# feiyeha/BS-YOLO

Measured on AMD Instinct MI355X. Metric: images/sec YOLO11s 640x640 bs=64 (forward + NMS), higher is better.
Workload: dtype f16

## Files before the change

bs_yolo_amd/csrc/conv_kernels.h:

```cpp
#pragma once
#include "common.h"

struct ConvK {
    const half_t* src0;
    const half_t* src1;
    int ld0, ld1, C0, C1, up0, up1;
    int H, W, OH, OW, stride, pad;
    int M;
    int Cin8;
    int ntaps;
    int nk;
    int Kpad;
    const half_t* wgt;
    const float* bias;
    void* dst;
    int ldd, Cout, out_f32;
    const half_t* res;
    int ldr;
    int act;
    int dst_scale, dst_dy, dst_dx;
    int ntn;
    int ntm;
    int tiles_x, tiles_y, B;
    int epi, y_f32, A, a0, nrows, raw_f32, rawC;
    float lvl_stride;
    int xyxy;
    void* y;
    void* raw;
    const half_t* tail_wgt;
    const float* tail_bias;
    unsigned span0, span1, wspan;
    int nsl_c, nsl_t, cb_per, taps_per, ldw;
    float* split_ws;
    long long slab;
    int korder;
};

__device__ __forceinline__ void dma16(const void* g, half_t* lds_wave_base) {
#if defined(__HIP_DEVICE_COMPILE__)
    __builtin_amdgcn_global_load_lds(g, lds_wave_base, 16, 0, 0);
#else
    (void)g;
    (void)lds_wave_base;
#endif
}

#if defined(__HIP_DEVICE_COMPILE__)
__device__ __forceinline__ void dma16_buf(bsy_rsrc_t r, unsigned voff, unsigned soff, half_t* lds_wave_base) {
    __builtin_amdgcn_raw_ptr_buffer_load_lds(r, lds_wave_base, 16, (int)voff, (int)soff, 0, 0);
}
#else
__device__ __forceinline__ void dma16_buf(bsy_rsrc_t, unsigned, unsigned, half_t*) {}
#endif

template <int MT, int NT>
__device__ __forceinline__ void conv_epilogue(const ConvK& p, f32x16 (&acc)[NT][MT], int m0, int n0, int wm, int wn,
                                              int lrow, int lh) {
    const int ohw = p.OH * p.OW;
    const bool wide = !p.out_f32 && !(p.Cout & 15) && !(p.ldd & 7) && !((uintptr_t)p.dst & 15);
#pragma unroll
    for (int b = 0; b < MT; ++b) {
        const int m = m0 + (wm * MT + b) * 32 + lrow;
        const bool mvalid = m < p.M;
        size_t dpix = (size_t)(mvalid ? m : 0);
        if (p.dst_scale != 1) {
            const int mm = mvalid ? m : 0;
            const int n = mm / ohw;
            const int rem = mm - n * ohw;
            const int oh = rem / p.OW;
            const int ow = rem - oh * p.OW;
            dpix = ((size_t)n * (p.OH * p.dst_scale) + (oh * p.dst_scale + p.dst_dy)) * (size_t)(p.OW * p.dst_scale) +
                   (ow * p.dst_scale + p.dst_dx);
        }
#pragma unroll
        for (int a = 0; a < NT; ++a) {
            const int cbase = n0 + (wn * NT + a) * 32;
            if (cbase >= p.Cout) continue;
            if (wide) {
                unsigned pk[4][2];
#pragma unroll
                for (int g = 0; g < 4; ++g) {
                    const int c = cbase + 8 * g + 4 * lh;
                    float v[4] = {0.f, 0.f, 0.f, 0.f};
                    if (c < p.Cout) {
#pragma unroll
                        for (int e = 0; e < 4; ++e) {
                            float t = acc[a][b][4 * g + e];
                            v[e] = p.act ? silu_f(t) : t;
                        }
                        if (p.res && mvalid) {
                            const half4 rv = *reinterpret_cast<const half4*>(p.res + dpix * p.ldr + c);
#pragma unroll
                            for (int e = 0; e < 4; ++e) v[e] += (float)rv[e];
                        }
                    }
                    half2v h0 = {(half_t)v[0], (half_t)v[1]}, h1 = {(half_t)v[2], (half_t)v[3]};
                    pk[g][0] = __builtin_bit_cast(unsigned, h0);
                    pk[g][1] = __builtin_bit_cast(unsigned, h1);
                }
#pragma unroll
                for (int g = 0; g < 4; g += 2) {
                    const auto r0 = __builtin_amdgcn_permlane32_swap(pk[g][0], pk[g + 1][0], false, false);
                    const auto r1 = __builtin_amdgcn_permlane32_swap(pk[g][1], pk[g + 1][1], false, false);
                    const int c = cbase + 8 * (g + lh);
                    if (mvalid && c < p.Cout) {
                        uint4 o = {r0[0], r1[0], r0[1], r1[1]};
                        *reinterpret_cast<uint4*>(reinterpret_cast<half_t*>(p.dst) + dpix * p.ldd + c) = o;
                    }
                }
                continue;
            }
            if (!mvalid) continue;
#pragma unroll
            for (int g = 0; g < 4; ++g) {
                const int c = cbase + 8 * g + 4 * lh;
                if (c >= p.Cout) continue;
                float v[4];
#pragma unroll
                for (int e = 0; e < 4; ++e) {
                    float t = acc[a][b][4 * g + e];
                    if (p.act) t = silu_f(t);
                    v[e] = t;
                }
                const bool full = c + 3 < p.Cout;
                if (p.res) {
                    const half_t* rp = p.res + dpix * p.ldr + c;
                    if (full) {
                        const half4 rv = *reinterpret_cast<const half4*>(rp);
#pragma unroll
                        for (int e = 0; e < 4; ++e) v[e] += (float)rv[e];
                    } else {
#pragma unroll
                        for (int e = 0; e < 4; ++e)
                            if (c + e < p.Cout) v[e] += (float)rp[e];
                    }
                }
                if (p.out_f32) {
                    float* dp = reinterpret_cast<float*>(p.dst) + dpix * p.ldd + c;
                    if (full) {
                        f32x4 o = {v[0], v[1], v[2], v[3]};
                        *reinterpret_cast<f32x4*>(dp) = o;
                    } else {
#pragma unroll
                        for (int e = 0; e < 4; ++e)
                            if (c + e < p.Cout) dp[e] = v[e];
                    }
                } else {
                    half_t* dp = reinterpret_cast<half_t*>(p.dst) + dpix * p.ldd + c;
                    if (full) {
                        half4 o = {(half_t)v[0], (half_t)v[1], (half_t)v[2], (half_t)v[3]};
                        *reinterpret_cast<half4*>(dp) = o;
                    } else {
#pragma unroll
                        for (int e = 0; e < 4; ++e)
                            if (c + e < p.Cout) dp[e] = (half_t)v[e];
                    }
                }
            }
        }
    }
}

template <typename T>
__device__ __forceinline__ void head_store(void* base, size_t idx, float v) { reinterpret_cast<T*>(base)[idx] = (T)v; }

__device__ __forceinline__ void dfl_decode_store(const ConvK& p, const f32x16& lo, const f32x16& hi, bool mv,
                                                 size_t ybase, size_t rbase, int pix, int lh) {
    const int hw = p.OH * p.OW;
    float dist[4];
#pragma unroll
    for (int sd = 0; sd < 4; ++sd) {
        const int rb = 8 * (sd & 1);
        float v[8];
#pragma unroll
        for (int g = 0; g < 2; ++g)
#pragma unroll
            for (int e = 0; e < 4; ++e) v[4 * g + e] = ((sd >> 1) ? hi : lo)[rb + 4 * g + e];
        if (p.raw && mv) {
#pragma unroll
            for (int i = 0; i < 8; ++i) {
                const size_t ri = rbase + (size_t)(16 * sd + (i & 3) + 8 * (i >> 2) + 4 * lh) * hw;
                if (p.raw_f32) head_store<float>(p.raw, ri, v[i]); else head_store<half_t>(p.raw, ri, v[i]);
            }
        }
        float mx = v[0];
#pragma unroll
        for (int i = 1; i < 8; ++i) mx = fmaxf(mx, v[i]);
        mx = fmaxf(mx, __shfl_xor(mx, 32, 64));
        float den = 0.f, num = 0.f;
#pragma unroll
        for (int i = 0; i < 8; ++i) {
            const float ex = __expf(v[i] - mx);
            den += ex;
            num += ex * (float)((i & 3) + 8 * (i >> 2) + 4 * lh);
        }
        den += __shfl_xor(den, 32, 64);
        num += __shfl_xor(num, 32, 64);
        dist[sd] = num / den;
    }
    if (mv && lh == 0) {
        const int ay_i = pix / p.OW, ax_i = pix - ay_i * p.OW;
        const float ax = (float)ax_i + 0.5f, ay = (float)ay_i + 0.5f;
        const float x1 = ax - dist[0], y1 = ay - dist[1], x2 = ax + dist[2], y2 = ay + dist[3];
        const float o[4] = {(p.xyxy ? x1 : (x1 + x2) * 0.5f) * p.lvl_stride, (p.xyxy ? y1 : (y1 + y2) * 0.5f) * p.lvl_stride,
                            (p.xyxy ? x2 : x2 - x1) * p.lvl_stride, (p.xyxy ? y2 : y2 - y1) * p.lvl_stride};
#pragma unroll
        for (int r = 0; r < 4; ++r) {
            const size_t yi = ybase + (size_t)r * p.A;
            if (p.y_f32) head_store<float>(p.y, yi, o[r]); else head_store<half_t>(p.y, yi, o[r]);
        }
    }
}

template <int MT, int NT>
__device__ __forceinline__ void conv_epilogue_head(const ConvK& p, f32x16 (&acc)[NT][MT], int m0, int n0, int wm, int wn,
                                                   int lrow, int lh) {
    const int hw = p.OH * p.OW;
#pragma unroll
    for (int b = 0; b < MT; ++b) {
        const int m = m0 + (wm * MT + b) * 32 + lrow;
        const bool mv = m < p.M;
        const int mm = mv ? m : 0;
        const int n = mm / hw, pix = mm - n * hw;
        const size_t ybase = (size_t)n * p.nrows * p.A + p.a0 + pix;
        const size_t rbase = (size_t)n * p.rawC * hw + pix;
        if (p.epi == 2) {
#pragma unroll
            for (int a = 0; a < NT; ++a) {
                const int cl = n0 + (wn * NT + a) * 32;
                if (cl >= p.Cout) continue;
#pragma unroll
                for (int g = 0; g < 4; ++g) {
                    const int c0 = cl + 8 * g + 4 * lh;
#pragma unroll
                    for (int e = 0; e < 4; ++e) {
                        const int c = c0 + e;
                        if (!mv || c >= p.Cout) continue;
                        const float v = acc[a][b][4 * g + e];
                        const float sg = sigmoid_f(v);
                        const size_t yi = ybase + (size_t)(4 + c) * p.A;
                        if (p.y_f32) head_store<float>(p.y, yi, sg); else head_store<half_t>(p.y, yi, sg);
                        if (p.raw) {
                            const size_t ri = rbase + (size_t)(64 + c) * hw;
                            if (p.raw_f32) head_store<float>(p.raw, ri, v); else head_store<half_t>(p.raw, ri, v);
                        }
                    }
                }
            }
        } else if (NT == 2) {
            dfl_decode_store(p, acc[0][b], acc[NT - 1][b], mv, ybase, rbase, pix, lh);
        }
    }
}

template <int TM, int TN, int MT, int NT, int NTHR>
__device__ __forceinline__ void conv_epilogue_cls_lds(const ConvK& p, f32x16 (&acc)[NT][MT], half_t* stile, int m0, int n0,
                                                      int wm, int wn, int lrow, int lh, int tid) {
    constexpr int LDP = TM + 8;
#pragma unroll
    for (int b = 0; b < MT; ++b) {
        const int prow = (wm * MT + b) * 32 + lrow;
#pragma unroll
        for (int a = 0; a < NT; ++a) {
            const int cl = (wn * NT + a) * 32;
            if (n0 + cl >= p.Cout) continue;
#pragma unroll
            for (int g = 0; g < 4; ++g) {
                const int c = cl + 8 * g + 4 * lh;
#pragma unroll
                for (int e = 0; e < 4; ++e) {
                    const float v = acc[a][b][4 * g + e];
                    stile[(c + e) * LDP + prow] = (half_t)sigmoid_f(v);
                }
            }
        }
    }
    __syncthreads();
    const int hw = p.OH * p.OW;
    half_t* y = reinterpret_cast<half_t*>(p.y);
    constexpr int GPR = TM / 8;
    for (int id = tid; id < TN * GPR; id += NTHR) {
        const int cr = id / GPR, g8 = (id - cr * GPR) * 8;
        const int c = n0 + cr, m = m0 + g8;
        if (c >= p.Cout || m >= p.M) continue;
        const int n = m / hw, pix = m - n * hw;
        const size_t yi = ((size_t)n * p.nrows + 4 + c) * p.A + p.a0 + pix;
        if (pix + 8 <= hw && m + 8 <= p.M && !(yi & 7)) {
            *reinterpret_cast<half8*>(y + yi) = *reinterpret_cast<const half8*>(stile + cr * LDP + g8);
        } else {
            for (int e = 0; e < 8 && m + e < p.M; ++e) {
                const int me = m + e, ne = me / hw, pe = me - ne * hw;
                y[((size_t)ne * p.nrows + 4 + c) * p.A + p.a0 + pe] = stile[cr * LDP + g8 + e];
            }
        }
    }
}

template <int TM, int TN, int MT, int NT, int NTHR>
__device__ __forceinline__ void conv_epilogue_lds(const ConvK& p, f32x16 (&acc)[NT][MT], half_t* stile, int m0, int n0,
                                                  int wm, int wn, int lrow, int lh, int tid) {
    constexpr int LDT = TN + 8;
#pragma unroll
    for (int b = 0; b < MT; ++b) {
        const int prow = (wm * MT + b) * 32 + lrow;
#pragma unroll
        for (int a = 0; a < NT; ++a) {
            const int cl = (wn * NT + a) * 32;
#pragma unroll
            for (int g = 0; g < 4; ++g) {
                const int c = cl + 8 * g + 4 * lh;
                half4 o;
                f32x4 t = f32x4{acc[a][b][4 * g], acc[a][b][4 * g + 1], acc[a][b][4 * g + 2], acc[a][b][4 * g + 3]};
                if (p.act) t = silu4_f(t);
#pragma unroll
                for (int e = 0; e < 4; ++e) o[e] = (half_t)t[e];
                *reinterpret_cast<half4*>(stile + prow * LDT + c) = o;
            }
        }
    }
    __syncthreads();
    constexpr int CPRW = TN / 8;
    constexpr int ITER = TM * CPRW / NTHR;
    half_t* dst = reinterpret_cast<half_t*>(p.dst);
#pragma unroll
    for (int i = 0; i < ITER; ++i) {
        const int id = tid + NTHR * i;
        const int row = id / CPRW, cc = (id % CPRW) * 8;
        const int m = m0 + row, c = n0 + cc;
        if (m >= p.M || c >= p.Cout) continue;
        half8 v = *reinterpret_cast<const half8*>(stile + row * LDT + cc);
        if (p.res) {
            const half8 r = *reinterpret_cast<const half8*>(p.res + (size_t)m * p.ldr + c);
#pragma unroll
            for (int e = 0; e < 8; ++e) v[e] = (half_t)((float)v[e] + (float)r[e]);
        }
        *reinterpret_cast<half8*>(dst + (size_t)m * p.ldd + c) = v;
    }
}

int launch_gemm_cfg(int id, int ksize, const ConvK& k, hipStream_t s);
int launch_stream1x1_cfg(int id, const ConvK& k, hipStream_t s);
int launch_patch_cfg(int id, bool tail, const ConvK& k, hipStream_t s);

constexpr int PERSIST_MAX_COUT = 1024;
```

bs_yolo_amd/csrc/conv_select.hip:

```cpp
#include <stdlib.h>

#include "conv_kernels.h"

extern "C" int bsy_conv_packed_dims(int C2, int C1, int ksize, int* cout_pad, int* k_pad) {
    if (C2 <= 0 || C1 <= 0 || (ksize != 1 && ksize != 3)) BSY_FAIL(BSY_ERR_ARG, "conv_packed_dims: bad shape");
    if (cout_pad) *cout_pad = round_up(C2, 128);
    if (C1 == 3) C1 = 4;
    if (k_pad) *k_pad = round_up(ksize * ksize * C1, 32);
    return BSY_OK;
}

int conv_korder(const ConvArgs& a) {
    const int Cin = a.C0 + a.C1;
    if (a.ksize != 3 || (Cin & 31) || (a.C0 & 31)) return 0;
    return (a.stride == 2 && !(Cin & 63) && !(a.C0 & 63)) ? 2 : 1;
}

enum ConvFam { CONV_GEMM, CONV_PERSIST, CONV_WRES, CONV_PATCH, CONV_TAIL };
struct ConvCfg {
    int id; ConvFam fam;
    int tm, tn, stages, bk;
    bool aligned;
    int tw, nfr;
};
template <int WM, int WN, int MT, int NT, int S, bool AL, int BK> constexpr ConvCfg gemm_row(int id) {
    return {id, CONV_GEMM, WM * MT * 32, WN * NT * 32, S, BK, AL, 0, 0};
}
template <int WM, int WN, int MT, int NT, int S, int BK> constexpr ConvCfg persist_row(int id) {
    return {id, CONV_PERSIST, WM * MT * 32, WN * NT * 32, S, BK, true, 0, 0};
}
template <int NT, int S, int NFR> constexpr ConvCfg wres_row(int id) {
    return {id, CONV_WRES, 128, 64 * NT, S, 32, true, 0, NFR};
}
template <int NT, int S, int TW, bool TAIL = false> constexpr ConvCfg patch_row(int id) {
    return {id, TAIL ? CONV_TAIL : CONV_PATCH, TW == 16 ? 8 * 16 : 6 * 20, 64 * NT, S, 32, true, TW, 0};
}
static const ConvCfg kConvCfgs[] = {
    gemm_row<4, 1, 2, 1, 3, false, 32>(0x00),
    gemm_row<4, 1, 2, 1, 3, true, 32>(0x01),
    gemm_row<4, 1, 2, 1, 2, true, 32>(0x02),
    gemm_row<4, 1, 2, 1, 2, true, 64>(0x03),
    gemm_row<4, 1, 2, 2, 3, false, 32>(0x10),
    gemm_row<4, 1, 2, 2, 3, true, 32>(0x11),
    gemm_row<4, 1, 2, 2, 2, true, 32>(0x12),
    gemm_row<4, 1, 2, 2, 2, true, 64>(0x13),
    gemm_row<2, 2, 2, 2, 3, false, 32>(0x20),
    gemm_row<2, 2, 2, 2, 3, true, 32>(0x21),
    gemm_row<2, 2, 2, 2, 2, true, 32>(0x22),
    gemm_row<2, 2, 2, 2, 2, true, 64>(0x23),
    gemm_row<2, 2, 2, 1, 3, false, 32>(0x30),
    gemm_row<2, 2, 2, 1, 3, true, 32>(0x31),
    gemm_row<2, 2, 2, 1, 2, true, 32>(0x32),
    gemm_row<2, 2, 2, 1, 2, true, 64>(0x33),
    gemm_row<4, 2, 2, 2, 3, true, 32>(0x41),
    gemm_row<4, 2, 2, 2, 2, true, 32>(0x42),
    gemm_row<4, 2, 2, 2, 2, true, 64>(0x43),
    gemm_row<1, 4, 2, 1, 3, false, 32>(0x50),
    gemm_row<1, 4, 2, 1, 3, true, 32>(0x51),
    gemm_row<1, 4, 2, 1, 2, true, 32>(0x52),
    gemm_row<1, 4, 2, 1, 2, true, 64>(0x53),
    gemm_row<2, 2, 1, 1, 3, false, 32>(0x60),
    gemm_row<2, 2, 1, 1, 3, true, 32>(0x61),
    gemm_row<2, 2, 1, 1, 2, true, 32>(0x62),
    gemm_row<2, 2, 1, 1, 2, true, 64>(0x63),
    gemm_row<4, 2, 2, 4, 3, true, 32>(0x71),
    gemm_row<4, 2, 2, 4, 2, true, 32>(0x72),
    gemm_row<4, 2, 2, 4, 2, true, 64>(0x73),
    persist_row<2, 2, 2, 2, 3, 32>(0x81),
    persist_row<2, 2, 2, 2, 2, 32>(0x82),
    persist_row<2, 2, 2, 2, 2, 64>(0x83),
    persist_row<2, 2, 2, 1, 3, 32>(0x91),
    persist_row<2, 2, 2, 1, 2, 32>(0x92),
    persist_row<2, 2, 2, 1, 2, 64>(0x93),
    patch_row<2, 2, 16>(0xA1),
    patch_row<1, 3, 16>(0xB1),
    patch_row<1, 2, 16>(0xB2),
    patch_row<1, 4, 16>(0xB3),
    patch_row<2, 2, 20>(0xC1),
    patch_row<1, 3, 20>(0xD1),
    patch_row<1, 2, 20>(0xD2),
    patch_row<1, 4, 20>(0xD3),
    patch_row<1, 3, 16, true>(0xB1),
    patch_row<1, 2, 16, true>(0xB2),
    patch_row<1, 4, 16, true>(0xB3),
    patch_row<1, 3, 20, true>(0xD1),
    patch_row<1, 2, 20, true>(0xD2),
    patch_row<1, 4, 20, true>(0xD3),
    wres_row<2, 4, 24>(0xE1),
    wres_row<2, 3, 24>(0xE2),
    wres_row<1, 4, 32>(0xF1),
    wres_row<1, 3, 32>(0xF2),
};

static const ConvCfg* conv_cfg_row(int cfg, bool tail) {
    for (const ConvCfg& r : kConvCfgs) if (r.id == (cfg & ~4) && (r.fam == CONV_TAIL) == tail) return &r;
    return nullptr;
}

bool conv_cfg_valid(const ConvArgs& a, int cfg) {
    const ConvCfg* r = conv_cfg_row(cfg, a.tail_wgt != nullptr);
    if (!r) return false;
    const int Cin = a.C0 + a.C1, ko = conv_korder(a), nsl = a.nsl_c * a.nsl_t;
    const bool aligned = !(Cin & 31) && !(a.C0 & 31), aligned64 = !(Cin & 63) && !(a.C0 & 63);
    if ((r->aligned && !aligned) || (r->bk == 64 && !aligned64)) return false;
    if (r->fam == CONV_GEMM) {
        if (!(cfg & 4) != !ko) return false;
        if (ko && (!r->aligned || (ko == 1 && r->bk == 64))) return false;
        if (nsl > 1 && (!r->aligned || (Cin / (a.nsl_c > 0 ? a.nsl_c : 1)) % r->bk)) return false;
        if (a.epi == 3 && (r->tm != 256 || r->tn != 64)) return false;
        return r->tn != 256 || !(a.Cout & 255);
    }
    if ((cfg & 4) || nsl > 1 || (r->fam == CONV_TAIL ? (a.epi != 3 || a.Cout != 64 || a.res) : a.epi != 0)) return false;
    if (a.out_f32 || (a.Cout & 7) || (a.ldd & 7) || ((uintptr_t)a.dst & 15) || a.dst_scale > 1) return false;
    if (r->fam == CONV_PERSIST || r->fam == CONV_WRES) {
        if (a.ksize != 1 || a.stride != 1 || a.res) return false;
        if (r->fam == CONV_PERSIST) return a.Cout <= PERSIST_MAX_COUT;
        return (r->tn / 64) * (Cin / 16) <= r->nfr && Cin / 32 >= r->stages - 1 && (r->tn != 128 || a.Cout > 64);
    }
    return ko == 1 && a.ksize == 3 && a.stride == 1 && a.pad == 1 && !a.C1 && !a.up0 && (!a.res || (!(a.ldr & 7) && !((uintptr_t)a.res & 15))) &&
           (r->tn != 128 || a.Cout > 64);
}

static bool family_off(const char* env) { return getenv(env) != nullptr; }

int conv_candidates(const ConvArgs& a, int* out, int max_out) {
    const int Cin = a.C0 + a.C1;
    const bool aligned = !(Cin & 31) && !(a.C0 & 31), aligned64 = !(Cin & 63) && !(a.C0 & 63);
    const long long M = (long long)a.B * a.OH * a.OW;
    const int tile = a.epi == 3 ? 1 : (a.Cout > 64 ? 2 : (a.Cout > 32 ? 1 : 0));
    const int ko = conv_korder(a), km = ko ? 4 : 0;
    const bool t20 = ceil_div(a.W, 20) * ceil_div(a.H, 6) < ceil_div(a.W, 16) * ceil_div(a.H, 8);
    int n = 0;
    auto add = [&](int c) {
        for (int i = 0; i < n; ++i) if (out[i] == c) return;
        if (n < max_out && conv_cfg_valid(a, c)) out[n++] = c;
    };
    if (a.tail_wgt) {
        if (t20) { add(0xD2); add(0xD1); add(0xD3); }
        add(0xB2); add(0xB1); add(0xB3); add(0xD2); add(0xD1); add(0xD3);
        return n;
    }
    if (!aligned) {
        add(tile << 4);
        if (a.Cout > 32) { add(0x30); add(0x60); }
        if (a.Cout > 64) add(0x50);
        return n;
    }
    const bool patch_ok = !family_off("BSY_NO_PATCH");
    if (!a.epi && a.ksize == 3 && a.stride == 1 && a.H >= 16 && a.W >= 16 && patch_ok) add(t20 ? 0xD2 : 0xB2);
    const int vbest = (aligned64 && ko != 1) ? 3 : 1;
    if (!a.epi && !(a.Cout & 255) && aligned64 && ko != 1 && M >= 16384) add(0x73 | km);
    add(tile << 4 | vbest | km);
    for (const ConvCfg& r : kConvCfgs) {
        if ((r.fam != CONV_GEMM && r.fam != CONV_PERSIST) || !r.aligned) continue;
        if (r.tn >= 2 * round_up(a.Cout, 32)) continue;
        if (r.tn == 32 && a.Cout > 32) continue;
        if (r.tm == 256 && r.tn == 128 && (a.Cout < 128 || M < 32768)) continue;
        if (r.tn == 256 && M < 16384) continue;
        if (r.fam == CONV_PERSIST && (M < 65536 || family_off("BSY_NO_PERSIST"))) continue;
        add(r.id | (r.fam == CONV_GEMM ? km : 0));
    }
    if (a.ksize == 1 && M >= 65536 && !family_off("BSY_NO_WRES"))
        for (const ConvCfg& r : kConvCfgs) if (r.fam == CONV_WRES) add(r.id);
    if (a.H >= 16 && a.W >= 16 && patch_ok)
        for (const ConvCfg& r : kConvCfgs) if (r.fam == CONV_PATCH && (r.tw == 16 || t20)) add(r.id);
    return n;
}

int launch_conv(const ConvArgs& a, hipStream_t s) {
    const int Cin = a.C0 + a.C1;
    if (a.ksize != 1 && a.ksize != 3) BSY_FAIL(BSY_ERR_ARG, "conv: ksize %d unsupported", a.ksize);
    if (a.stride != 1 && a.stride != 2) BSY_FAIL(BSY_ERR_ARG, "conv: stride %d unsupported", a.stride);
    if ((a.C0 & 7) || (a.C1 & 7) || (a.ld0 & 7) || (a.C1 && (a.ld1 & 7)))
        BSY_FAIL(BSY_ERR_ARG, "conv: channel counts/strides must be multiples of 8 (C0=%d C1=%d ld0=%d ld1=%d)", a.C0,
                 a.C1, a.ld0, a.ld1);
    if ((a.ldd & 3) || (a.res && (a.ldr & 3))) BSY_FAIL(BSY_ERR_ARG, "conv: dst/res row stride must be a multiple of 4");
    if (((uintptr_t)a.src0 & 15) || ((uintptr_t)a.src1 & 15) || ((uintptr_t)a.wgt & 15) || ((uintptr_t)a.bias & 15) ||
        ((uintptr_t)a.dst & 7) || ((uintptr_t)a.res & 7))
        BSY_FAIL(BSY_ERR_ARG, "conv: misaligned pointer");
    if (a.C1 && !a.src1) BSY_FAIL(BSY_ERR_ARG, "conv: src1 missing");
    if ((a.up0 && ((a.H | a.W) & 1)) || (a.up1 && ((a.H | a.W) & 1))) BSY_FAIL(BSY_ERR_ARG, "conv: odd size with upsample");
    if (a.OH != (a.H + 2 * a.pad - a.ksize) / a.stride + 1 || a.OW != (a.W + 2 * a.pad - a.ksize) / a.stride + 1)
        BSY_FAIL(BSY_ERR_ARG, "conv: output extent mismatch");
    const long long M = (long long)a.B * a.OH * a.OW;
    if (M <= 0 || M > 0x7fffffffLL) BSY_FAIL(BSY_ERR_ARG, "conv: M out of range");
    if (a.epi) {
        if ((a.epi != 2 && a.epi != 3) || !a.y || a.A <= 0 || a.a0 < 0 || a.a0 + a.OH * a.OW > a.A || a.dst_scale > 1 || a.res)
            BSY_FAIL(BSY_ERR_ARG, "conv: bad fused-decoder arguments (epi %d)", a.epi);
        if (a.epi == 3 && (a.Cout != 64 || a.nrows < 4)) BSY_FAIL(BSY_ERR_ARG, "conv: DFL epilogue needs 64 box channels");
        if (a.tail_wgt && (a.epi != 3 || !a.tail_bias || a.ksize != 3 || ((uintptr_t)a.tail_wgt & 15) || ((uintptr_t)a.tail_bias & 15)))
            BSY_FAIL(BSY_ERR_ARG, "conv: bad box-branch tail arguments");
        if (a.epi == 2 && a.nrows < 4 + a.Cout) BSY_FAIL(BSY_ERR_ARG, "conv: y has %d rows, class epilogue needs %d", a.nrows, 4 + a.Cout);
        if (a.raw && a.rawC < (a.epi == 3 ? 64 : 64 + a.Cout)) BSY_FAIL(BSY_ERR_ARG, "conv: raw map has too few channels");
    }
    ConvK k;
    k.src0 = a.src0; k.src1 = a.src1; k.ld0 = a.ld0; k.ld1 = a.ld1; k.C0 = a.C0; k.C1 = a.C1;
    k.up0 = a.up0; k.up1 = a.up1; k.H = a.H; k.W = a.W; k.OH = a.OH; k.OW = a.OW; k.stride = a.stride; k.pad = a.pad;
    k.M = (int)M; k.Cin8 = Cin / 8; k.ntaps = a.ksize * a.ksize;
    k.Kpad = round_up(a.ksize * a.ksize * Cin, 32); k.nk = k.Kpad / 32;
    k.wgt = a.wgt; k.bias = a.bias; k.dst = a.dst; k.ldd = a.ldd; k.Cout = a.Cout; k.out_f32 = a.out_f32;
    k.res = a.res; k.ldr = a.ldr; k.act = a.act; k.B = a.B; k.tiles_x = k.tiles_y = 0;
    k.epi = a.epi; k.y = a.y; k.y_f32 = a.y_f32; k.A = a.A; k.a0 = a.a0; k.nrows = a.nrows; k.lvl_stride = a.lvl_stride;
    k.xyxy = a.epi == 3 && a.xyxy;
    k.raw = a.raw; k.raw_f32 = a.raw_f32; k.rawC = a.rawC;
    k.tail_wgt = a.tail_wgt; k.tail_bias = a.tail_bias;
    if (a.tail_wgt && !a.epi) BSY_FAIL(BSY_ERR_ARG, "conv: a box-branch tail needs the decoder arguments (epi 3)");
    k.dst_scale = a.dst_scale > 0 ? a.dst_scale : 1; k.dst_dy = a.dst_dy; k.dst_dx = a.dst_dx; k.ntn = 1;
    k.nsl_c = k.nsl_t = 1; k.cb_per = Cin; k.taps_per = a.ksize * a.ksize; k.split_ws = nullptr; k.slab = 0; k.ldw = 0;
    if (a.nsl_c * a.nsl_t > 1) {
        const int nt = a.ksize * a.ksize;
        if (a.nsl_c < 1 || a.nsl_t < 1 || !a.split_ws || a.epi || a.out_f32 || a.tail_wgt || (a.dst_scale > 1) || (Cin % a.nsl_c) || ((Cin / a.nsl_c) & 31) || (a.C0 & 31) ||
            (nt % a.nsl_t) || (a.Cout & 7) || (a.ldd & 7) || ((uintptr_t)a.dst & 15) || (a.res && ((a.ldr & 7) || ((uintptr_t)a.res & 15))) || ((uintptr_t)a.split_ws & 15))
            BSY_FAIL(BSY_ERR_ARG, "conv: bad split-K arguments (%d x %d slices)", a.nsl_c, a.nsl_t);
        if (conv_korder(a) == 2 && ((Cin / a.nsl_c) & 63)) BSY_FAIL(BSY_ERR_ARG, "conv: split-K slices of a 64-channel-chunk layer must be multiples of 64 channels");
        k.nsl_c = a.nsl_c; k.nsl_t = a.nsl_t; k.cb_per = Cin / a.nsl_c; k.taps_per = nt / a.nsl_t; k.split_ws = a.split_ws;
        k.ldw = round_up(a.Cout, 32);
        k.slab = (long long)M * k.ldw;
    }
    if (a.ksize == 3 && (a.up0 || a.up1)) BSY_FAIL(BSY_ERR_ARG, "conv: upsampled source only with ksize 1");
    if ((long long)a.B * a.H * a.W * (long long)(a.ld0 > a.ld1 ? a.ld0 : a.ld1) >= (1LL << 31))
        BSY_FAIL(BSY_ERR_ARG, "conv: source view exceeds 2^31 elements (split the batch)");
    {
        const long long px0 = (long long)a.B * (a.H >> a.up0) * (a.W >> a.up0), px1 = (long long)a.B * (a.H >> a.up1) * (a.W >> a.up1);
        k.span0 = (unsigned)(((px0 - 1) * a.ld0 + a.C0) * 2);
        k.span1 = a.C1 ? (unsigned)(((px1 - 1) * a.ld1 + a.C1) * 2) : 0u;
        k.wspan = (unsigned)((long long)round_up(a.Cout, 128) * k.Kpad * 2);
    }
    int cfg = a.cfg;
    if (cfg < 0 || !conv_cfg_valid(a, cfg)) {
        int list[BSY_CONV_MAX_CFG];
        if (conv_candidates(a, list, BSY_CONV_MAX_CFG) <= 0) BSY_FAIL(BSY_ERR_ARG, "conv: no kernel configuration for this shape");
        cfg = list[0];
    }
    k.korder = conv_korder(a);
    const ConvCfg* r = conv_cfg_row(cfg, a.tail_wgt != nullptr);
    switch (r->fam) {
        case CONV_GEMM: return launch_gemm_cfg(r->id, a.ksize, k, s);
        case CONV_PERSIST:
        case CONV_WRES: return launch_stream1x1_cfg(r->id, k, s);
        case CONV_PATCH:
        case CONV_TAIL: return launch_patch_cfg(r->id, r->fam == CONV_TAIL, k, s);
    }
    BSY_FAIL(BSY_ERR_ARG, "conv: configuration 0x%02x has no kernel family", cfg);
}
```

bs_yolo_amd/csrc/conv_stream1x1.hip:

```cpp
#include "conv_kernels.h"

template <int WAVES_M, int WAVES_N, int MT, int NT, int STAGES, int BK>
__global__ __launch_bounds__(512) void conv1x1_persist_kernel(const ConvK p) {
    constexpr int TM = WAVES_M * MT * 32, TN = WAVES_N * NT * 32;
    constexpr int TNS = TN < 64 ? 64 : TN;
    constexpr int CPR = BK / 8, RPI = 64 / CPR;
    constexpr int PIW = TM / (RPI * 4), WIW = TNS / (RPI * 4);
    constexpr int STAGE = (TM + TNS) * BK, NDMA = PIW + WIW;
    constexpr int SWS = BK == 32 ? 2 : 1;
    constexpr int LDT = TN + 8, OT = TM * LDT;
    static_assert(WAVES_M * WAVES_N == 4 && PIW >= 1 && WIW >= 1 && (BK == 32 || (!(PIW & 1) && !(WIW & 1))), "bad tile");
    __shared__ __attribute__((aligned(16))) half_t smem[STAGES * STAGE + OT + 2 * PERSIST_MAX_COUT];
    half_t* otile = smem + STAGES * STAGE;
    float* sbias = reinterpret_cast<float*>(otile + OT);

    const int tid = threadIdx.x, lane = tid & 63;
    const int wave = __builtin_amdgcn_readfirstlane(tid >> 6);
    const int nk = p.Kpad / BK;
    const int ntiles = p.ntm * p.ntn;
    const TileWalk tw = xcd_tile_walk(blockIdx.x, gridDim.x, ntiles);
    const int T0 = tw.tile, G = tw.step;
    const int my_tiles = T0 < tw.end ? (tw.end - T0 + G - 1) / G : 0;
    for (int i = tid; i < p.ntn * TN; i += 512) sbias[i] = p.bias[i];
    __syncthreads();

    if (wave >= 4) {
        const int st = tid - 256;
        constexpr int CPRW = TN / 8, ITER = TM * CPRW / 256;
        half_t* dst = reinterpret_cast<half_t*>(p.dst);
        for (int t = 0; t < my_tiles; ++t) {
            const int tile = T0 + t * G;
            const int m0 = (tile / p.ntn) * TM, n0 = (tile % p.ntn) * TN;
            for (int k = 0; k < nk; ++k) __builtin_amdgcn_s_barrier();
            __builtin_amdgcn_s_barrier();
            half8 v[ITER];
#pragma unroll
            for (int i = 0; i < ITER; ++i) {
                const int id = st + 256 * i;
                v[i] = *reinterpret_cast<const half8*>(otile + (id / CPRW) * LDT + (id % CPRW) * 8);
            }
#pragma unroll
            for (int i = 0; i < ITER; ++i) {
                const int id = st + 256 * i;
                const int m = m0 + id / CPRW, c = n0 + (id % CPRW) * 8;
                if (m < p.M && c < p.Cout) *reinterpret_cast<half8*>(dst + (size_t)m * p.ldd + c) = v[i];
            }
        }
        return;
    }

    const int wm = wave / WAVES_N, wn = wave % WAVES_N;
    const int rsub = lane / CPR, slot = lane % CPR;
    const int kc0 = BK == 32 ? (slot ^ ((rsub >> 2) & 3)) : (slot ^ (rsub >> 1));
    const int kc1 = BK == 32 ? kc0 : (slot ^ (4 | (rsub >> 1)));
    const bsy_rsrc_t rs0 = make_rsrc(p.src0, p.span0), rs1 = make_rsrc(p.src1 ? p.src1 : p.src0, p.src1 ? p.span1 : 0u),
                     rsw = make_rsrc(p.wgt, p.wspan);
    const int ohw = p.OH * p.OW;
    const int Cin = p.Cin8 * 8;

    unsigned off0[PIW], off1[PIW], woff[WIW];
    bool rv[PIW];
    int it = 0, ikt = 0, s_cb = 0;
    auto setup_tile = [&](int tcount) {
        const int tile = T0 + tcount * G;
        const int m0 = (tile / p.ntn) * TM, n0 = (tile % p.ntn) * TN;
#pragma unroll
        for (int i = 0; i < PIW; ++i) {
            const int m = m0 + (wave * PIW + i) * RPI + rsub;
            rv[i] = m < p.M;
            const int mm = rv[i] ? m : 0;
            if (!(p.up0 | p.up1) && p.stride == 1) {
                off0[i] = (unsigned)mm * (unsigned)p.ld0;
                off1[i] = (unsigned)mm * (unsigned)p.ld1;
            } else {
                const int n = mm / ohw, rem = mm - n * ohw, oh = rem / p.OW, ow = rem - oh * p.OW;
                const int iy = oh * p.stride, ix = ow * p.stride;
                const int H0 = p.H >> p.up0, W0 = p.W >> p.up0, H1 = p.H >> p.up1, W1 = p.W >> p.up1;
                off0[i] = (unsigned)((n * H0 + (iy >> p.up0)) * W0 + (ix >> p.up0)) * (unsigned)p.ld0;
                off1[i] = (unsigned)((n * H1 + (iy >> p.up1)) * W1 + (ix >> p.up1)) * (unsigned)p.ld1;
            }
        }
#pragma unroll
        for (int j = 0; j < WIW; ++j)
            woff[j] = (unsigned)(n0 + (wave * WIW + j) * RPI + rsub) * (unsigned)p.Kpad + ((j & 1) ? kc1 : kc0) * 8;
        s_cb = 0;
    };
    auto issue_step = [&](int stage) {
        if (ikt == 0) setup_tile(it);
        half_t* sP = smem + stage * STAGE;
        half_t* sW = sP + TM * BK;
        const bool s1 = s_cb >= p.C0;
        const unsigned sc = 2u * (unsigned)(s1 ? s_cb - p.C0 : s_cb);
#pragma unroll
        for (int i = 0; i < PIW; ++i) {
            const unsigned kcb = 16u * (unsigned)((i & 1) ? kc1 : kc0);
            const unsigned o = rv[i] ? 2u * (s1 ? off1[i] : off0[i]) + sc + kcb : BSY_OOB;
            if (s1) dma16_buf(rs1, o, 0u, sP + (wave * PIW + i) * RPI * BK);
            else dma16_buf(rs0, o, 0u, sP + (wave * PIW + i) * RPI * BK);
        }
#pragma unroll
        for (int j = 0; j < WIW; ++j)
            dma16_buf(rsw, 2u * woff[j], (unsigned)ikt * (2u * BK), sW + (wave * WIW + j) * RPI * BK);
        s_cb += BK;
        if (++ikt == nk) { ikt = 0; ++it; }
    };

    const int lrow = lane & 31, lh = lane >> 5;
    f32x16 acc[NT][MT];
#pragma unroll
    for (int a = 0; a < NT; ++a)
#pragma unroll
        for (int b = 0; b < MT; ++b) acc_bias(acc[a][b], sbias + (T0 % p.ntn) * TN + (wn * NT + a) * 32, lh);
    const int total = my_tiles * nk;
    int ip = 0;
    for (; ip < STAGES - 1 && ip < total; ++ip) issue_step(ip % STAGES);
    int ckt = 0, ct = 0;
    for (int cp = 0; cp < total; ++cp) {
        const int later = min(STAGES - 2, total - 1 - cp);
        if (later >= STAGES - 2 && STAGES > 2) {
            asm volatile("s_waitcnt vmcnt(%0)" ::"n"((STAGES - 2) * NDMA) : "memory");
        } else {
            asm volatile("s_waitcnt vmcnt(0)" ::: "memory");
        }
        __builtin_amdgcn_s_barrier();
        if (ip < total) { issue_step(ip % STAGES); ++ip; }
        const half_t* sP = smem + (cp % STAGES) * STAGE;
        const half_t* sW = sP + TM * BK;
        constexpr int KSUB = BK / 16;
        half8 bfr[KSUB][MT], afr[KSUB][NT];
#pragma unroll
        for (int ks = 0; ks < KSUB; ++ks) {
            const int chunk = 2 * ks + lh;
#pragma unroll
            for (int b = 0; b < MT; ++b) {
                const int row = (wm * MT + b) * 32 + lrow;
                bfr[ks][b] = *reinterpret_cast<const half8*>(sP + row * BK + ((chunk ^ ((row >> SWS) & (CPR - 1))) << 3));
            }
#pragma unroll
            for (int a = 0; a < NT; ++a) {
                const int row = (wn * NT + a) * 32 + lrow;
                afr[ks][a] = *reinterpret_cast<const half8*>(sW + row * BK + ((chunk ^ ((row >> SWS) & (CPR - 1))) << 3));
            }
        }
        __builtin_amdgcn_sched_barrier(0);
#pragma unroll
        for (int ks = 0; ks < KSUB; ++ks)
#pragma unroll
            for (int a = 0; a < NT; ++a)
#pragma unroll
                for (int b = 0; b < MT; ++b)
                    acc[a][b] = __builtin_amdgcn_mfma_f32_32x32x16_f16(afr[ks][a], bfr[ks][b], acc[a][b], 0, 0, 0);
        if (++ckt == nk) {
            ckt = 0;
            const int n1 = ((T0 + (ct + 1) * G) % p.ntn) * TN;
#pragma unroll
            for (int b = 0; b < MT; ++b) {
                const int prow = (wm * MT + b) * 32 + lrow;
#pragma unroll
                for (int a = 0; a < NT; ++a) {
                    const int cl = (wn * NT + a) * 32;
#pragma unroll
                    for (int g = 0; g < 4; ++g) {
                        const int c = cl + 8 * g + 4 * lh;
                        const f32x4 bn = *reinterpret_cast<const f32x4*>(sbias + n1 + c);
                        half4 o;
                        f32x4 tv = f32x4{acc[a][b][4 * g], acc[a][b][4 * g + 1], acc[a][b][4 * g + 2], acc[a][b][4 * g + 3]};
                        if (p.act) tv = silu4_f(tv);
#pragma unroll
                        for (int e = 0; e < 4; ++e) {
                            o[e] = (half_t)tv[e];
                            acc[a][b][4 * g + e] = bn[e];
                        }
                        *reinterpret_cast<half4*>(otile + prow * LDT + c) = o;
                    }
                }
            }
            asm volatile("s_waitcnt lgkmcnt(0)" ::: "memory");
            __builtin_amdgcn_s_barrier();
            ++ct;
        }
    }
}

template <int WM, int WN, int MT, int NT, int STAGES, int BK>
static int launch_persist(const ConvK& k, hipStream_t s) {
    constexpr int TM = WM * MT * 32, TN = WN * NT * 32;
    ConvK p = k;
    p.ntn = ceil_div(k.Cout, TN);
    p.ntm = ceil_div(k.M, TM);
    const long long ntiles = (long long)p.ntm * p.ntn;
    if (ntiles <= 0 || ntiles > 0x7fffffffLL) BSY_FAIL(BSY_ERR_ARG, "conv: tile count %lld out of range", ntiles);
    constexpr int lds_bytes = ((TM + (TN < 64 ? 64 : TN)) * BK * STAGES + TM * (TN + 8) + 2 * PERSIST_MAX_COUT) * 2;
    const int per_cu = 160 * 1024 / lds_bytes > 2 ? 2 : (160 * 1024 / lds_bytes);
    const long long grid = ntiles < 256LL * per_cu ? ntiles : 256LL * per_cu;
    hipLaunchKernelGGL((conv1x1_persist_kernel<WM, WN, MT, NT, STAGES, BK>), dim3((unsigned)grid), dim3(512), 0, s, p);
    HIP_TRY(hipGetLastError());
    return BSY_OK;
}

template <int NT, int STAGES, int NFR>
__global__ __launch_bounds__(256, 2) void conv1x1_wres_kernel(const ConvK p) {
    constexpr int BK = 32, MT = 2, TM = 128, TN = 64 * NT;
    constexpr int CPR = 4, RPI = 16;
    constexpr int PIW = TM / (RPI * 4);
    constexpr int STAGE = TM * BK;
    constexpr int LDT = TN + 8, OT = TM * LDT;
    constexpr int CPRW = TN / 8, NST = TM * CPRW / 256;
    __shared__ __attribute__((aligned(16))) half_t smem[STAGES * STAGE + OT + 2 * TN];
    half_t* otile = smem + STAGES * STAGE;
    float* sbias = reinterpret_cast<float*>(otile + OT);

    const int tid = threadIdx.x, lane = tid & 63;
    const int wave = __builtin_amdgcn_readfirstlane(tid >> 6);
    const int wm = wave >> 1, wn = wave & 1;
    const int lrow = lane & 31, lh = lane >> 5;
    const int nk = p.Kpad / BK;
    constexpr int X = 8;
    const int x = blockIdx.x % X, q = blockIdx.x / X;
    const int ct = q % p.ntn, slot = q / p.ntn;
    const int walkers = (gridDim.x / X) / p.ntn;
    const int per = p.ntm / X, rem = p.ntm % X;
    const int pt0 = x * per + (x < rem ? x : rem), ptn = per + (x < rem ? 1 : 0);
    const int my_tiles = slot < ptn ? (ptn - slot + walkers - 1) / walkers : 0;
    const int n0 = ct * TN;

    half8 afr[NFR];
    const int nfr = nk * 2 * NT;
#pragma unroll
    for (int i = 0; i < NFR; ++i) {
        afr[i] = half8{0, 0, 0, 0, 0, 0, 0, 0};
        if (i < nfr) {
            const int ks = i / NT, a = i - ks * NT;
            afr[i] = *reinterpret_cast<const half8*>(p.wgt + (size_t)(n0 + (wn * NT + a) * 32 + lrow) * p.Kpad + 16 * ks + 8 * lh);
        }
    }
    if (tid < TN) sbias[tid] = p.bias[n0 + tid];
    asm volatile("s_waitcnt vmcnt(0)" ::: "memory");
    __syncthreads();

    const int rsub = lane / CPR, slot4 = lane % CPR;
    const int kc = slot4 ^ ((rsub >> 2) & 3);
    const bsy_rsrc_t rs0 = make_rsrc(p.src0, p.span0), rs1 = make_rsrc(p.src1 ? p.src1 : p.src0, p.src1 ? p.span1 : 0u);
    const int ohw = p.OH * p.OW;
    unsigned off0[PIW], off1[PIW];
    bool rv[PIW];
    int it = 0, ikt = 0, s_cb = 0;
    auto setup_tile = [&](int tcount) {
        const int m0 = (pt0 + slot + tcount * walkers) * TM;
#pragma unroll
        for (int i = 0; i < PIW; ++i) {
            const int m = m0 + (wave * PIW + i) * RPI + rsub;
            rv[i] = m < p.M;
            const int mm = rv[i] ? m : 0;
            if (!(p.up0 | p.up1)) {
                off0[i] = (unsigned)mm * (unsigned)p.ld0;
                off1[i] = (unsigned)mm * (unsigned)p.ld1;
            } else {
                const int n = mm / ohw, r2 = mm - n * ohw, oh = r2 / p.OW, ow = r2 - oh * p.OW;
                const int H0 = p.H >> p.up0, W0 = p.W >> p.up0, H1 = p.H >> p.up1, W1 = p.W >> p.up1;
                off0[i] = (unsigned)((n * H0 + (oh >> p.up0)) * W0 + (ow >> p.up0)) * (unsigned)p.ld0;
                off1[i] = (unsigned)((n * H1 + (oh >> p.up1)) * W1 + (ow >> p.up1)) * (unsigned)p.ld1;
            }
        }
        s_cb = 0;
    };
    auto issue_step = [&](int stage) {
        if (ikt == 0) setup_tile(it);
        half_t* sP = smem + stage * STAGE;
        const bool s1 = s_cb >= p.C0;
        const unsigned sc = 2u * (unsigned)(s1 ? s_cb - p.C0 : s_cb) + 16u * (unsigned)kc;
#pragma unroll
        for (int i = 0; i < PIW; ++i) {
            const unsigned o = rv[i] ? 2u * (s1 ? off1[i] : off0[i]) + sc : BSY_OOB;
            if (s1) dma16_buf(rs1, o, 0u, sP + (wave * PIW + i) * RPI * BK);
            else dma16_buf(rs0, o, 0u, sP + (wave * PIW + i) * RPI * BK);
        }
        s_cb += BK;
        if (++ikt == nk) { ikt = 0; ++it; }
    };

    f32x16 acc[NT][MT];
#pragma unroll
    for (int a = 0; a < NT; ++a)
#pragma unroll
        for (int b = 0; b < MT; ++b) acc_bias(acc[a][b], sbias + (wn * NT + a) * 32, lh);
    const int total = my_tiles * nk;
    int ip = 0;
    for (; ip < STAGES - 1 && ip < total; ++ip) issue_step(ip % STAGES);
    int ckt = 0, ct_done = 0;
    half_t* dst = reinterpret_cast<half_t*>(p.dst);
    for (int cp = 0; cp < total; ++cp) {
        const int later = min(STAGES - 2, total - 1 - cp);
        const bool st_young = ct_done > 0 && ckt < STAGES - 1;
        if (later >= STAGES - 2) {
            if (st_young) asm volatile("s_waitcnt vmcnt(%0)" ::"n"((STAGES - 2) * PIW + NST) : "memory");
            else asm volatile("s_waitcnt vmcnt(%0)" ::"n"((STAGES - 2) * PIW) : "memory");
        } else {
            asm volatile("s_waitcnt vmcnt(0)" ::: "memory");
        }
        __builtin_amdgcn_s_barrier();
        if (ip < total) { issue_step(ip % STAGES); ++ip; }
        const half_t* sP = smem + (cp % STAGES) * STAGE;
#pragma unroll
        for (int ks = 0; ks < 2; ++ks) {
            const int chunk = 2 * ks + lh;
            half8 bfr[MT];
#pragma unroll
            for (int b = 0; b < MT; ++b) {
                const int row = (wm * MT + b) * 32 + lrow;
                bfr[b] = *reinterpret_cast<const half8*>(sP + row * BK + ((chunk ^ ((row >> 2) & 3)) << 3));
            }
#pragma unroll
            for (int kk = 0; kk < NFR / (2 * NT); ++kk)
                if (kk == ckt) {
#pragma unroll
                    for (int a = 0; a < NT; ++a)
#pragma unroll
                        for (int b = 0; b < MT; ++b)
                            acc[a][b] = __builtin_amdgcn_mfma_f32_32x32x16_f16(afr[(2 * kk + ks) * NT + a], bfr[b], acc[a][b], 0, 0, 0);
                }
        }
        if (++ckt == nk) {
            ckt = 0;
            const int m0 = (pt0 + slot + ct_done * walkers) * TM;
#pragma unroll
            for (int b = 0; b < MT; ++b) {
                const int prow = (wm * MT + b) * 32 + lrow;
#pragma unroll
                for (int a = 0; a < NT; ++a)
#pragma unroll
                    for (int g = 0; g < 4; ++g) {
                        const int c = (wn * NT + a) * 32 + 8 * g + 4 * lh;
                        half4 o;
                        const f32x4 bn = *reinterpret_cast<const f32x4*>(sbias + c);
                        f32x4 tv = f32x4{acc[a][b][4 * g], acc[a][b][4 * g + 1], acc[a][b][4 * g + 2], acc[a][b][4 * g + 3]};
                        if (p.act) tv = silu4_f(tv);
#pragma unroll
                        for (int e = 0; e < 4; ++e) {
                            o[e] = (half_t)tv[e];
                            acc[a][b][4 * g + e] = bn[e];
                        }
                        *reinterpret_cast<half4*>(otile + prow * LDT + c) = o;
                    }
            }
            asm volatile("s_waitcnt lgkmcnt(0)" ::: "memory");
            __builtin_amdgcn_s_barrier();
            half8 v[NST];
#pragma unroll
            for (int i = 0; i < NST; ++i) {
                const int id = tid + 256 * i;
                v[i] = *reinterpret_cast<const half8*>(otile + (id / CPRW) * LDT + (id % CPRW) * 8);
            }
#pragma unroll
            for (int i = 0; i < NST; ++i) {
                const int id = tid + 256 * i;
                const int m = m0 + id / CPRW, c = n0 + (id % CPRW) * 8;
                if (m < p.M && c < p.Cout) *reinterpret_cast<half8*>(dst + (size_t)m * p.ldd + c) = v[i];
            }
            ++ct_done;
        }
    }
}

template <int NT, int STAGES, int NFR>
static int launch_wres(const ConvK& k, hipStream_t s) {
    constexpr int TM = 128, TN = 64 * NT;
    ConvK p = k;
    p.ntn = ceil_div(k.Cout, TN);
    p.ntm = ceil_div(k.M, TM);
    int grid = 512 / (8 * p.ntn) * (8 * p.ntn);
    if (grid < 8 * p.ntn) grid = 8 * p.ntn;
    const int walkers_per_xcd = grid / 8 / p.ntn;
    if (walkers_per_xcd > ceil_div(p.ntm, 8)) grid = 8 * p.ntn * (ceil_div(p.ntm, 8) > 0 ? ceil_div(p.ntm, 8) : 1);
    hipLaunchKernelGGL((conv1x1_wres_kernel<NT, STAGES, NFR>), dim3((unsigned)grid), dim3(256), 0, s, p);
    HIP_TRY(hipGetLastError());
    return BSY_OK;
}

template <int NT, int S, int NFR> static int launch_wres_nfr(const ConvK& k, hipStream_t s) {
    return NT * ((k.C0 + k.C1) / 16) <= 16 ? launch_wres<NT, S, 16>(k, s) : launch_wres<NT, S, NFR>(k, s);
}

int launch_stream1x1_cfg(int id, const ConvK& k, hipStream_t s) {
    switch (id) {
        case 0x81: return launch_persist<2, 2, 2, 2, 3, 32>(k, s);
        case 0x82: return launch_persist<2, 2, 2, 2, 2, 32>(k, s);
        case 0x83: return launch_persist<2, 2, 2, 2, 2, 64>(k, s);
        case 0x91: return launch_persist<2, 2, 2, 1, 3, 32>(k, s);
        case 0x92: return launch_persist<2, 2, 2, 1, 2, 32>(k, s);
        case 0x93: return launch_persist<2, 2, 2, 1, 2, 64>(k, s);
        case 0xE1: return launch_wres_nfr<2, 4, 24>(k, s);
        case 0xE2: return launch_wres_nfr<2, 3, 24>(k, s);
        case 0xF1: return launch_wres_nfr<1, 4, 32>(k, s);
        case 0xF2: return launch_wres_nfr<1, 3, 32>(k, s);
    }
    BSY_FAIL(BSY_ERR_ARG, "conv: no streaming 1x1 kernel is built for configuration 0x%02x", id);
}
```

Baseline: 21880.

## Fuse class-score sigmoid decode into weights-resident 1x1 conv kernel

```diff
diff --git a/bs_yolo_amd/csrc/conv_kernels.h b/bs_yolo_amd/csrc/conv_kernels.h
--- a/bs_yolo_amd/csrc/conv_kernels.h
+++ b/bs_yolo_amd/csrc/conv_kernels.h
@@ -343,3 +343,4 @@
 int launch_patch_cfg(int id, bool tail, const ConvK& k, hipStream_t s);
 
 constexpr int PERSIST_MAX_COUT = 1024;
+constexpr int WRES_CLS_NFR = 16;
diff --git a/bs_yolo_amd/csrc/conv_select.hip b/bs_yolo_amd/csrc/conv_select.hip
--- a/bs_yolo_amd/csrc/conv_select.hip
+++ b/bs_yolo_amd/csrc/conv_select.hip
@@ -110,7 +110,12 @@
         if (a.epi == 3 && (r->tm != 256 || r->tn != 64)) return false;
         return r->tn != 256 || !(a.Cout & 255);
     }
-    if ((cfg & 4) || nsl > 1 || (r->fam == CONV_TAIL ? (a.epi != 3 || a.Cout != 64 || a.res) : a.epi != 0)) return false;
+    if ((cfg & 4) || nsl > 1) return false;
+    if (r->fam == CONV_WRES && a.epi == 2) {
+        if (a.y_f32 || a.raw || !a.y || ((uintptr_t)a.y & 15) || a.ksize != 1 || a.stride != 1 || a.res || Cin < 128) return false;
+        return (r->tn / 64) * (Cin / 16) <= WRES_CLS_NFR && Cin / 32 >= r->stages - 1 && (r->tn != 128 || a.Cout > 64);
+    }
+    if (r->fam == CONV_TAIL ? (a.epi != 3 || a.Cout != 64 || a.res) : a.epi != 0) return false;
     if (a.out_f32 || (a.Cout & 7) || (a.ldd & 7) || ((uintptr_t)a.dst & 15) || a.dst_scale > 1) return false;
     if (r->fam == CONV_PERSIST || r->fam == CONV_WRES) {
         if (a.ksize != 1 || a.stride != 1 || a.res) return false;
@@ -150,6 +155,7 @@
     if (!a.epi && a.ksize == 3 && a.stride == 1 && a.H >= 16 && a.W >= 16 && patch_ok) add(t20 ? 0xD2 : 0xB2);
     const int vbest = (aligned64 && ko != 1) ? 3 : 1;
     if (!a.epi && !(a.Cout & 255) && aligned64 && ko != 1 && M >= 16384) add(0x73 | km);
+    if (a.epi == 2 && a.ksize == 1 && Cin == 128 && a.OH * a.OW >= 6400 && M >= 65536 && !family_off("BSY_NO_WRES")) add(a.Cout > 64 ? 0xE2 : 0xF2);
     add(tile << 4 | vbest | km);
     for (const ConvCfg& r : kConvCfgs) {
         if ((r.fam != CONV_GEMM && r.fam != CONV_PERSIST) || !r.aligned) continue;
diff --git a/bs_yolo_amd/csrc/conv_stream1x1.hip b/bs_yolo_amd/csrc/conv_stream1x1.hip
--- a/bs_yolo_amd/csrc/conv_stream1x1.hip
+++ b/bs_yolo_amd/csrc/conv_stream1x1.hip
@@ -190,6 +190,7 @@
     p.ntm = ceil_div(k.M, TM);
     const long long ntiles = (long long)p.ntm * p.ntn;
     if (ntiles <= 0 || ntiles > 0x7fffffffLL) BSY_FAIL(BSY_ERR_ARG, "conv: tile count %lld out of range", ntiles);
+    if (k.epi) BSY_FAIL(BSY_ERR_ARG, "conv: the persistent 1x1 kernel has no fused decoder (epi %d)", k.epi);
     constexpr int lds_bytes = ((TM + (TN < 64 ? 64 : TN)) * BK * STAGES + TM * (TN + 8) + 2 * PERSIST_MAX_COUT) * 2;
     const int per_cu = 160 * 1024 / lds_bytes > 2 ? 2 : (160 * 1024 / lds_bytes);
     const long long grid = ntiles < 256LL * per_cu ? ntiles : 256LL * per_cu;
@@ -198,14 +199,23 @@
     return BSY_OK;
 }
 
-template <int NT, int STAGES, int NFR>
+
+template <int BASE, int NMAX> __device__ __forceinline__ void wait_vm_counted(int n) {
+    static_assert(BASE + NMAX <= 63, "vmcnt is a 6-bit field");
+#pragma unroll
+    for (int k = 0; k <= NMAX; ++k)
+        if (n == k) asm volatile("s_waitcnt vmcnt(%0)" ::"n"(BASE + k) : "memory");
+}
+template <int NT, int STAGES, int NFR, bool CLS>
 __global__ __launch_bounds__(256, 2) void conv1x1_wres_kernel(const ConvK p) {
     constexpr int BK = 32, MT = 2, TM = 128, TN = 64 * NT;
     constexpr int CPR = 4, RPI = 16;
     constexpr int PIW = TM / (RPI * 4);
     constexpr int STAGE = TM * BK;
-    constexpr int LDT = TN + 8, OT = TM * LDT;
+    constexpr int LDT = TN + 8, LDP = TM + 8;
+    constexpr int OT = CLS && TN * LDP > TM * LDT ? TN * LDP : TM * LDT;
     constexpr int CPRW = TN / 8, NST = TM * CPRW / 256;
+    constexpr int GPR = TM / 8, NSTC = TN * GPR / 256;
     __shared__ __attribute__((aligned(16))) half_t smem[STAGES * STAGE + OT + 2 * TN];
     half_t* otile = smem + STAGES * STAGE;
     float* sbias = reinterpret_cast<float*>(otile + OT);
@@ -288,12 +298,14 @@
     int ip = 0;
     for (; ip < STAGES - 1 && ip < total; ++ip) issue_step(ip % STAGES);
     int ckt = 0, ct_done = 0;
+    int prev_st = 0;
     half_t* dst = reinterpret_cast<half_t*>(p.dst);
     for (int cp = 0; cp < total; ++cp) {
         const int later = min(STAGES - 2, total - 1 - cp);
         const bool st_young = ct_done > 0 && ckt < STAGES - 1;
         if (later >= STAGES - 2) {
-            if (st_young) asm volatile("s_waitcnt vmcnt(%0)" ::"n"((STAGES - 2) * PIW + NST) : "memory");
+            if (CLS && st_young && prev_st >= 0) wait_vm_counted<(STAGES - 2) * PIW, NSTC>(prev_st);
+            else if (!CLS && st_young) asm volatile("s_waitcnt vmcnt(%0)" ::"n"((STAGES - 2) * PIW + NST) : "memory");
             else asm volatile("s_waitcnt vmcnt(%0)" ::"n"((STAGES - 2) * PIW) : "memory");
         } else {
             asm volatile("s_waitcnt vmcnt(0)" ::: "memory");
@@ -323,6 +335,63 @@
         if (++ckt == nk) {
             ckt = 0;
             const int m0 = (pt0 + slot + ct_done * walkers) * TM;
+            if constexpr (CLS) {
+#pragma unroll
+                for (int b = 0; b < MT; ++b) {
+                    const int prow = (wm * MT + b) * 32 + lrow;
+#pragma unroll
+                    for (int a = 0; a < NT; ++a) {
+                        const int cl = (wn * NT + a) * 32;
+                        if (n0 + cl >= p.Cout) continue;
+#pragma unroll
+                        for (int g = 0; g < 4; ++g) {
+                            const int c = cl + 8 * g + 4 * lh;
+                            const f32x4 bn = *reinterpret_cast<const f32x4*>(sbias + c);
+#pragma unroll
+                            for (int e = 0; e < 4; ++e) {
+                                otile[(c + e) * LDP + prow] = (half_t)sigmoid_f(acc[a][b][4 * g + e]);
+                                acc[a][b][4 * g + e] = bn[e];
+                            }
+                        }
+                    }
+                }
+                asm volatile("s_waitcnt lgkmcnt(0)" ::: "memory");
+                __builtin_amdgcn_s_barrier();
+                const int hw = p.OH * p.OW;
+                half_t* y = reinterpret_cast<half_t*>(p.y);
+                half8 v[NSTC];
+#pragma unroll
+                for (int i = 0; i < NSTC; ++i) {
+                    const int id = tid + 256 * i;
+                    v[i] = *reinterpret_cast<const half8*>(otile + (id / GPR) * LDP + (id % GPR) * 8);
+                }
+                int nst = 0;
+                bool single = false;
+#pragma unroll
+                for (int i = 0; i < NSTC; ++i) {
+                    const int id = tid + 256 * i;
+                    const int c = n0 + id / GPR, m = m0 + (id % GPR) * 8;
+                    const bool live = c < p.Cout && m < p.M;
+                    const int n = m / hw, pix = m - n * hw;
+                    const size_t yi = ((size_t)n * p.nrows + 4 + c) * p.A + p.a0 + pix;
+                    const bool whole = live && pix + 8 <= hw && m + 8 <= p.M && !(yi & 7);
+                    if (whole) *reinterpret_cast<half8*>(y + yi) = v[i];
+                    nst += __any(whole) ? 1 : 0;
+                    if (__any(live && !whole)) {
+                        single = true;
+                        if (live && !whole) {
+#pragma unroll
+                            for (int e = 0; e < 8; ++e) {
+                                const int me = m + e, ne = me / hw, pe = me - ne * hw;
+                                if (me < p.M) y[((size_t)ne * p.nrows + 4 + c) * p.A + p.a0 + pe] = v[i][e];
+                            }
+                        }
+                    }
+                }
+                prev_st = __builtin_amdgcn_readfirstlane(single ? -1 : nst);
+                ++ct_done;
+                continue;
+            }
 #pragma unroll
             for (int b = 0; b < MT; ++b) {
                 const int prow = (wm * MT + b) * 32 + lrow;
@@ -372,7 +441,14 @@
     if (grid < 8 * p.ntn) grid = 8 * p.ntn;
     const int walkers_per_xcd = grid / 8 / p.ntn;
     if (walkers_per_xcd > ceil_div(p.ntm, 8)) grid = 8 * p.ntn * (ceil_div(p.ntm, 8) > 0 ? ceil_div(p.ntm, 8) : 1);
-    hipLaunchKernelGGL((conv1x1_wres_kernel<NT, STAGES, NFR>), dim3((unsigned)grid), dim3(256), 0, s, p);
+    if (k.epi && (k.epi != 2 || k.y_f32 || k.raw || !k.y || ((uintptr_t)k.y & 15)))
+        BSY_FAIL(BSY_ERR_ARG, "conv: the weights-resident 1x1 kernel decodes f16 class scores only (epi %d)", k.epi);
+    if (k.epi) {
+        if constexpr (NFR <= WRES_CLS_NFR) hipLaunchKernelGGL((conv1x1_wres_kernel<NT, STAGES, NFR, true>), dim3((unsigned)grid), dim3(256), 0, s, p);
+        else BSY_FAIL(BSY_ERR_ARG, "conv: the class-score form of the weights-resident 1x1 kernel holds %d fragments at most", WRES_CLS_NFR);
+    } else {
+        hipLaunchKernelGGL((conv1x1_wres_kernel<NT, STAGES, NFR, false>), dim3((unsigned)grid), dim3(256), 0, s, p);
+    }
     HIP_TRY(hipGetLastError());
     return BSY_OK;
 }
```

Measured after the change: 21900 (median of 3 runs). About the same (+0.1%).
